# e4s2022/e4s

Measured on AMD Instinct MI355X. Metric: 1024^2 face-swap images/sec, higher is better.
Workload: dtype f32 operands as hi+lo bf16, 3 bf16 MFMAs per product, f32 accumulate (bf16x3) on the 3x3 convs whose launch fills the chip; exact f32 elsewhere; 1 GPU; E4S-core face swap at 1024^2 (2x Net3 encoder @256^2, style swap, 12 LocalMLPs, mask-guided StyleGAN2 generator K=13), BASELINE.json configs[3] shard: 8 swaps per GPU per step; per_gpu_batch=8, global_batch=8, out_size=1024, hip_graph=True, precision=as bf16x3 where the launch fills the chip (this batch), else exact fp32, parallelism=image-parallel x1

## Files before the change

e4s_amd/build.py:

```python
import hashlib
import os
import subprocess
import sys

HERE = os.path.dirname(os.path.abspath(__file__))
ROOT = os.path.dirname(HERE)
CSRC = os.path.join(HERE, "csrc")
LIB = os.path.join(HERE, "libe4s_hip.so")
STAMP = os.path.join(HERE, ".libe4s_hip.stamp")
ARCH = "gfx950"


def sources():
    return sorted(os.path.join(CSRC, f) for f in os.listdir(CSRC) if f.endswith(".hip"))


PER_FILE_FLAGS = {"conv_region1w.hip": ["-fno-slp-vectorize"], "conv_wino1w.hip": ["-fno-slp-vectorize"],
                  "conv_gather1w.hip": ["-fno-slp-vectorize"]}


def _extra_flags():
    flags = ["-DE4S_ABLATIONS"] if os.environ.get("E4S_BUILD_ABLATIONS") == "1" else []
    return flags + os.environ.get("E4S_EXTRA_CFLAGS", "").split()


def _digest():
    h = hashlib.sha256()
    h.update(" ".join(_extra_flags()).encode())
    h.update(repr(sorted(PER_FILE_FLAGS.items())).encode())
    headers = sorted(os.path.join(CSRC, f) for f in os.listdir(CSRC) if f.endswith(".h"))
    files = sources() + headers + [os.path.join(ROOT, "include", "e4s_hip.h")]
    for f in files:
        h.update(f.encode())
        with open(f, "rb") as fh:
            h.update(fh.read())
    return h.hexdigest()


def _compile_and_link(lib, objdir, verbose):
    hipcc = os.environ.get("HIPCC", "/opt/rocm/bin/hipcc")
    if not os.path.isfile(hipcc):
        hipcc = "hipcc"
    os.makedirs(objdir, exist_ok=True)
    procs, objs = [], []
    for src in sources():
        obj = os.path.join(objdir, os.path.basename(src) + ".o")
        cmd = [hipcc, f"--offload-arch={ARCH}", "-O3", "-std=c++17", "-fPIC", "-I" + os.path.join(ROOT, "include"),
               "-I" + CSRC] + _extra_flags() + PER_FILE_FLAGS.get(os.path.basename(src), []) + ["-c", src, "-o", obj]
        if verbose:
            print(" ".join(cmd), flush=True)
        procs.append((src, subprocess.Popen(cmd, stdout=subprocess.PIPE, stderr=subprocess.STDOUT)))
        objs.append(obj)
    for src, pr in procs:
        out, _ = pr.communicate()
        if pr.returncode != 0:
            sys.stderr.write(out.decode(errors="replace"))
            raise RuntimeError(f"hipcc failed on {src}")
    res = subprocess.run([hipcc, f"--offload-arch={ARCH}", "-shared", "-fPIC", "-o", lib] + objs, stdout=subprocess.PIPE, stderr=subprocess.STDOUT)
    if res.returncode != 0:
        sys.stderr.write(res.stdout.decode(errors="replace"))
        raise RuntimeError(f"link of {os.path.basename(lib)} failed")
    return lib


def build(force=False, verbose=False):
    alt = os.environ.get("E4S_BUILD_OUT")
    if alt:
        return _build_to(os.path.abspath(alt), os.path.join(os.path.dirname(os.path.abspath(alt)), "obj_" + os.path.basename(alt)), verbose)
    dig = _digest()
    if not force and os.path.isfile(LIB) and os.path.isfile(STAMP) and open(STAMP).read().strip() == dig:
        return LIB
    _compile_and_link(LIB, os.path.join(HERE, "build"), verbose)
    with open(STAMP, "w") as fh:
        fh.write(dig)
    return LIB


def _build_to(lib, objdir, verbose=False):
    return _compile_and_link(lib, objdir, verbose)


if __name__ == "__main__":
    print(build(force="--force" in sys.argv, verbose=True))
```

e4s_amd/csrc/upconv_bf16x3.hip:

```cpp
#include "conv_launch.h"
#include <stdlib.h>

namespace {


constexpr int PKC = 32;
constexpr int KC = 16, ROWB = 80, LO = 32;
constexpr int TAH = 8, TAW = 16;
constexpr int HH = TAH + 1, HW = TAW + 1, HALO = HH * HW;
constexpr int OH = 2 * TAH - 4, OW = 2 * TAW - 4;
constexpr int IQH = 2 * TAH, IQW = 2 * TAW;
constexpr int BNC = 32;
constexpr int NTHR = 256, NBLK = 9;
constexpr int ITEMS = HALO * 2;
constexpr int AJ = (ITEMS + NTHR - 1) / NTHR;
constexpr int BPIECES = NBLK * BNC * 4;
constexpr int BJ = (BPIECES + NTHR - 1) / NTHR;
constexpr int A_BYTES = HALO * ROWB;
constexpr int B_BYTES = NBLK * BNC * ROWB;
constexpr int STAGE_BYTES = 2 * A_BYTES + 2 * B_BYTES;
constexpr int I_BYTES = IQH * IQW * BNC * 4;
constexpr int NZ = OH * OW;
constexpr int MAXC = 512;
constexpr int SMEM = STAGE_BYTES + NZ * 4 + 2 * MAXC * 4;
static_assert(I_BYTES <= STAGE_BYTES, "the I tile aliases the stage buffers");
static_assert(2 * SMEM <= 160 * 1024, "two blocks per CU");
static_assert(8 * OW <= NTHR && NZ <= 2 * NTHR, "epilogue thread layout");

__device__ __forceinline__ void split_store(unsigned char* dst, const f32x8 v) {
    const bf16x8 h = __builtin_convertvector(v, bf16x8);
    const f32x8 r = v - __builtin_convertvector(h, f32x8);
    const bf16x8 l = __builtin_convertvector(r, bf16x8);
    *reinterpret_cast<bf16x8*>(dst) = h;
    *reinterpret_cast<bf16x8*>(dst + LO) = l;
}

struct TileId { int tb, ty, tx, nt; };

template <int XF, int PC = 0>
__global__ __launch_bounds__(NTHR, 2) void upconv_fused_kernel(const e4s_conv_params p, const float* __restrict__ k4, const int ntn,
                                                           const int tx_n, const int per_img, const int ntiles, const int abl_arg) {
#ifdef E4S_ABLATIONS
    const int abl = abl_arg;
#else
    constexpr int abl = 0;
#endif
    extern __shared__ __attribute__((aligned(16))) unsigned char smem[];
    unsigned char* sA = smem;
    unsigned char* sB = smem + 2 * A_BYTES;
    float* sI = reinterpret_cast<float*>(smem);
    float* s_nz = reinterpret_cast<float*>(smem + STAGE_BYTES);
    float* s_sty = s_nz + NZ;

    const int tid = threadIdx.x;
    const int lane = tid & 63, wm = __builtin_amdgcn_readfirstlane(tid >> 6);
    const int li = lane & 31, kh = lane >> 5;
    const int G = gridDim.x;
    const int first = xcd_remap(blockIdx.x, G);
    const int nchunk = p.Cin / KC;
    const unsigned char* wbytes = reinterpret_cast<const unsigned char*>(p.w);
    const size_t img_stride = (size_t)p.Hi * p.Wi * p.Cin;

    auto decode = [&](int t) -> TileId {
        TileId id;
        const int mt = t / ntn;
        id.nt = t - mt * ntn;
        id.tb = mt / per_img;
        const int rem = mt - id.tb * per_img;
        id.ty = rem / tx_n;
        id.tx = rem - id.ty * tx_n;
        return id;
    };
    auto item_src = [&](const TileId& id, int item, bool& ok) -> size_t {
        const int h = item >> 1, q = item & 1;
        const int hy = h / HW, hx = h - hy * HW;
        const int iy = id.ty * (OH / 2) - 2 + hy, ix = id.tx * (OW / 2) - 2 + hx;
        ok = item < ITEMS && (unsigned)iy < (unsigned)p.Hi && (unsigned)ix < (unsigned)p.Wi;
        return ok ? ((size_t)iy * p.Wi + ix) * p.Cin + q * 8 : (size_t)(q * 8);
    };
    auto item_dst = [&](int item) -> int { return (item >> 1) * ROWB + (item & 1) * 16; };
    const f32x8 zero8 = {0.f, 0.f, 0.f, 0.f, 0.f, 0.f, 0.f, 0.f};
    auto b_src = [&](int i, int c, int nt) -> size_t {
        return ((size_t)(c >> 1) * ntn + nt) * (NBLK * BNC * 128) + (size_t)(i >> 2) * 128 + ((i >> 1) & 1) * 64 + (c & 1) * 32 + (i & 1) * 16;
    };
    auto b_dst = [&](int i) -> int { return (i >> 2) * ROWB + (i & 3) * 16; };

    struct AReg {
        f32x8 a[AJ];
        bool ok[AJ];
    };
    typedef f32x4 BReg[BJ];
    auto fetch_a = [&](AReg& R, const TileId& id, int chunk, bool real) {
        const float* xb = p.x + (real ? (size_t)id.tb * img_stride + chunk * KC : 0);
#pragma unroll
        for (int j = 0; j < AJ; ++j) {
            const int item = tid + NTHR * j;
            const size_t off = item_src(id, item, R.ok[j]);
            if (abl != 4) R.a[j] = load8(xb + off);
        }
    };
    auto load_style = [&](const TileId& id, int par) {
        if (XF)
            for (int i = tid * 4; i < p.Cin; i += NTHR * 4)
                *reinterpret_cast<f32x4*>(s_sty + par * MAXC + i) = *reinterpret_cast<const f32x4*>(p.in_scale + (size_t)id.tb * p.Cin + i);
    };
    auto fetch_b = [&](BReg& R, const TileId& id, int chunk, bool real) {
#pragma unroll
        for (int j = 0; j < BJ; ++j) {
            const int i = tid + NTHR * j;
            if (abl != 4) R[j] = *reinterpret_cast<const f32x4*>(wbytes + b_src(i < BPIECES ? i : 0, real ? chunk : 0, real ? id.nt : 0));
        }
    };
    auto store_a = [&](const AReg& R, int buf, int chunk, int par) {
#pragma unroll
        for (int j = 0; j < AJ; ++j) {
            const int item = tid + NTHR * j;
            if (item < ITEMS) {
                f32x8 v = R.a[j];
                if (XF) v = v * load8(s_sty + par * MAXC + chunk * KC + (item & 1) * 8);
                if (!R.ok[j]) v = zero8;
                split_store(sA + buf * A_BYTES + item_dst(item), v);
            }
        }
    };
    auto store_b = [&](const BReg& R, int buf) {
#pragma unroll
        for (int j = 0; j < BJ; ++j) {
            const int i = tid + NTHR * j;
            if (i < BPIECES) *reinterpret_cast<f32x4*>(sB + buf * B_BYTES + b_dst(i)) = R[j];
        }
    };

    if (first >= ntiles) return;
    TileId cur = decode(first);
    int t_next = first + G;
    bool has_next = t_next < ntiles;
    TileId nxt = decode(has_next ? t_next : first);

    AReg RE, RO;
    BReg RB;
    int par = 0;
    fetch_a(RE, cur, 0, true);
    fetch_b(RB, cur, 0, true);
    load_style(cur, 0);
    if (XF) __syncthreads();
    store_a(RE, 0, 0, 0);
    store_b(RB, 0);
    fetch_a(RO, cur, 1, true);
    __syncthreads();

    const int m_row = wm * 32 + li;
    const int arow = ((m_row / TAW) * HW + (m_row % TAW)) * ROWB + kh * 16;
    const int brow = li * ROWB + kh * 16;
    const int e_c4 = tid & 7, e_ox = tid >> 3;
    const bool e_act = e_ox < OW;

    float fu[4], fv[4];
    bool sep;
    {
        float kk[16], vmax = 0.f;
#pragma unroll
        for (int a = 0; a < 16; ++a) {
            kk[a] = k4[a];
            vmax = fmaxf(vmax, fabsf(kk[a]));
        }
        sep = kk[0] != 0.f;
        const float inv = sep ? 1.f / kk[0] : 0.f;
#pragma unroll
        for (int i = 0; i < 4; ++i) {
            fu[3 - i] = kk[4 * i];
            fv[3 - i] = kk[i] * inv;
        }
#pragma unroll
        for (int i = 0; i < 4; ++i)
#pragma unroll
            for (int j = 0; j < 4; ++j) sep = sep && fabsf(kk[4 * i + j] - fu[3 - i] * fv[3 - j]) <= 1e-6f * vmax;
    }

    f32x16 acc[4];
    auto contract = [&](int buf) {
        const unsigned char* Ab = sA + buf * A_BYTES + arow;
        const unsigned char* Bb = sB + buf * B_BYTES + brow;
        struct Frag { bf16x8 h, l; };
        auto ldA = [&](int shift) -> Frag {
            const unsigned char* a = Ab + ((1 - (shift >> 1)) * HW + (1 - (shift & 1))) * ROWB;
            return Frag{*reinterpret_cast<const bf16x8*>(a), *reinterpret_cast<const bf16x8*>(a + LO)};
        };
        auto ldB = [&](int blk) -> Frag {
            const unsigned char* b = Bb + blk * (BNC * ROWB);
            return Frag{*reinterpret_cast<const bf16x8*>(b), *reinterpret_cast<const bf16x8*>(b + LO)};
        };
        {
            const Frag a0 = ldA(0), b0 = ldB(0), b4 = ldB(4), b6 = ldB(6), b8 = ldB(8);
            const Frag a1 = ldA(1), b1 = ldB(1), b7 = ldB(7);
            acc[0] = __builtin_amdgcn_mfma_f32_32x32x16_bf16(a0.l, b0.h, acc[0], 0, 0, 0);
            acc[1] = __builtin_amdgcn_mfma_f32_32x32x16_bf16(a0.l, b4.h, acc[1], 0, 0, 0);
            acc[2] = __builtin_amdgcn_mfma_f32_32x32x16_bf16(a0.l, b6.h, acc[2], 0, 0, 0);
            acc[3] = __builtin_amdgcn_mfma_f32_32x32x16_bf16(a0.l, b8.h, acc[3], 0, 0, 0);
            acc[0] = __builtin_amdgcn_mfma_f32_32x32x16_bf16(a0.h, b0.l, acc[0], 0, 0, 0);
            acc[1] = __builtin_amdgcn_mfma_f32_32x32x16_bf16(a0.h, b4.l, acc[1], 0, 0, 0);
            acc[2] = __builtin_amdgcn_mfma_f32_32x32x16_bf16(a0.h, b6.l, acc[2], 0, 0, 0);
            acc[3] = __builtin_amdgcn_mfma_f32_32x32x16_bf16(a0.h, b8.l, acc[3], 0, 0, 0);
            acc[0] = __builtin_amdgcn_mfma_f32_32x32x16_bf16(a0.h, b0.h, acc[0], 0, 0, 0);
            acc[1] = __builtin_amdgcn_mfma_f32_32x32x16_bf16(a0.h, b4.h, acc[1], 0, 0, 0);
            acc[2] = __builtin_amdgcn_mfma_f32_32x32x16_bf16(a0.h, b6.h, acc[2], 0, 0, 0);
            acc[3] = __builtin_amdgcn_mfma_f32_32x32x16_bf16(a0.h, b8.h, acc[3], 0, 0, 0);
            acc[0] = __builtin_amdgcn_mfma_f32_32x32x16_bf16(a1.l, b1.h, acc[0], 0, 0, 0);
            acc[2] = __builtin_amdgcn_mfma_f32_32x32x16_bf16(a1.l, b7.h, acc[2], 0, 0, 0);
            acc[0] = __builtin_amdgcn_mfma_f32_32x32x16_bf16(a1.h, b1.l, acc[0], 0, 0, 0);
            acc[2] = __builtin_amdgcn_mfma_f32_32x32x16_bf16(a1.h, b7.l, acc[2], 0, 0, 0);
            acc[0] = __builtin_amdgcn_mfma_f32_32x32x16_bf16(a1.h, b1.h, acc[0], 0, 0, 0);
            acc[2] = __builtin_amdgcn_mfma_f32_32x32x16_bf16(a1.h, b7.h, acc[2], 0, 0, 0);
        }
        {
            const Frag a2 = ldA(2), b2 = ldB(2), b5 = ldB(5);
            const Frag a3 = ldA(3), b3 = ldB(3);
            acc[0] = __builtin_amdgcn_mfma_f32_32x32x16_bf16(a2.l, b2.h, acc[0], 0, 0, 0);
            acc[1] = __builtin_amdgcn_mfma_f32_32x32x16_bf16(a2.l, b5.h, acc[1], 0, 0, 0);
            acc[0] = __builtin_amdgcn_mfma_f32_32x32x16_bf16(a2.h, b2.l, acc[0], 0, 0, 0);
            acc[1] = __builtin_amdgcn_mfma_f32_32x32x16_bf16(a2.h, b5.l, acc[1], 0, 0, 0);
            acc[0] = __builtin_amdgcn_mfma_f32_32x32x16_bf16(a2.h, b2.h, acc[0], 0, 0, 0);
            acc[1] = __builtin_amdgcn_mfma_f32_32x32x16_bf16(a2.h, b5.h, acc[1], 0, 0, 0);
            acc[0] = __builtin_amdgcn_mfma_f32_32x32x16_bf16(a3.l, b3.h, acc[0], 0, 0, 0);
            acc[0] = __builtin_amdgcn_mfma_f32_32x32x16_bf16(a3.h, b3.l, acc[0], 0, 0, 0);
            acc[0] = __builtin_amdgcn_mfma_f32_32x32x16_bf16(a3.h, b3.h, acc[0], 0, 0, 0);
        }
    };

    for (;;) {
        if (has_next) load_style(nxt, par ^ 1);
#pragma unroll
        for (int c = 0; c < 4; ++c)
#pragma unroll
            for (int r = 0; r < 16; ++r) acc[c][r] = 0.f;
        float nz_reg[2] = {0.f, 0.f};
        if (!PC && p.noise) {
#pragma unroll
            for (int j = 0; j < 2; ++j) {
                const int e = tid + NTHR * j;
                const int oy = cur.ty * OH + e / OW, ox = cur.tx * OW + e % OW;
                if (e < NZ && oy < p.Ho && ox < p.Wo) nz_reg[j] = p.noise[(int64_t)cur.tb * p.noise_bstride + (int64_t)oy * p.Wo + ox];
            }
        }
        f32x4 d_reg = {1.f, 1.f, 1.f, 1.f}, b_reg = {0.f, 0.f, 0.f, 0.f};
        if (e_act) {
            const int co0 = cur.nt * BNC + e_c4 * 4;
            if (p.out_scale) d_reg = *reinterpret_cast<const f32x4*>(p.out_scale + (size_t)cur.tb * p.Cout + co0);
            if (p.bias) b_reg = *reinterpret_cast<const f32x4*>(p.bias + co0);
        }
        const float nw_reg = p.noise ? p.noise_w[0] : 0.f;

        for (int c0 = 0; c0 < nchunk; c0 += 2) {
            const bool last_pair = (c0 + 2 == nchunk);
            const TileId& nid = last_pair ? nxt : cur;
            const bool nreal = !last_pair || has_next;
            const int ce = last_pair ? 0 : c0 + 2, co = last_pair ? 1 : c0 + 3;
            fetch_a(RE, nid, ce, nreal);
            fetch_b(RB, cur, c0 + 1, true);
            if (abl != 1) contract(0);
            if (abl != 5) {
                store_a(RO, 1, c0 + 1, par);
                store_b(RB, 1);
            }
            __syncthreads();
            fetch_a(RO, nid, co, nreal);
            fetch_b(RB, nid, ce, nreal);
            if (abl != 1) contract(1);
            if (!last_pair && abl != 5) {
                store_a(RE, 0, ce, par);
                store_b(RB, 0);
            }
            __syncthreads();
        }

#pragma unroll
        for (int j = 0; j < 2; ++j)
            if (!PC && tid + NTHR * j < NZ) s_nz[tid + NTHR * j] = nw_reg * nz_reg[j];
        if (abl == 3 || abl == 7) asm volatile("" :: "v"(acc[0][0]), "v"(acc[1][7]), "v"(acc[2][3]), "v"(acc[3][9]));
        if (abl != 3 && abl != 7)
#pragma unroll
        for (int cls = 0; cls < 4; ++cls) {
            const int dy = cls >> 1, dx = cls & 1;
#pragma unroll
            for (int r = 0; r < 16; ++r) {
                const int m = wm * 32 + (r & 3) + 8 * (r >> 2) + 4 * kh;
                const int qy = 2 * (m / TAW) + dy, qx = 2 * (m % TAW) + dx;
                sI[(qy * IQW + qx) * BNC + li] = acc[cls][r];
            }
        }
        __syncthreads();
        if (e_act && abl != 2 && abl != 3) {
            const int co0 = cur.nt * BNC + e_c4 * 4;
            const int ox = cur.tx * OW + e_ox;
            const f32x4 d = d_reg, bs = b_reg;
            const float gain = (p.act == 1) ? p.gain : 1.f;
            const int ycs = p.y_cstride ? p.y_cstride : p.Cout;
            const float* ip = sI + (IQW + e_ox + 1) * BNC + e_c4 * 4;
            auto finish = [&](f32x4 v, int r) {
                const int oy = cur.ty * OH + r;
                if (oy < p.Ho && ox < p.Wo) {
                    if (PC) {
                        const f32x4 nz = *reinterpret_cast<const f32x4*>(
                            p.noise + ((int64_t)cur.tb * p.noise_bstride + (int64_t)oy * p.Wo + ox) * p.Cout + co0);
                        f32x4 nzw;
#pragma unroll
                        for (int e = 0; e < 4; ++e) nzw[e] = e4s_mul_rn(nw_reg, nz[e]);
                        v = v * d + bs + nzw;
                    } else
                    v = v * d + bs + s_nz[r * OW + e_ox];
                    if (p.act) {
#pragma unroll
                        for (int e = 0; e < 4; ++e) v[e] = (v[e] > 0.f ? v[e] : v[e] * p.alpha) * gain;
                    }
                    f32x4* dst = reinterpret_cast<f32x4*>(p.y + (((size_t)cur.tb * p.Ho + oy) * p.Wo + ox) * ycs + co0);
                    if (abl == 6) asm volatile("" :: "v"(v));
                    else *dst = v;
                }
            };
            if (sep) {
                auto hrow = [&](int ry) -> f32x4 {
                    const float* q = ip + ry * IQW * BNC;
                    return *reinterpret_cast<const f32x4*>(q) * fv[0] + *reinterpret_cast<const f32x4*>(q + BNC) * fv[1] +
                           *reinterpret_cast<const f32x4*>(q + 2 * BNC) * fv[2] + *reinterpret_cast<const f32x4*>(q + 3 * BNC) * fv[3];
                };
                f32x4 h0 = hrow(0), h1 = hrow(1), h2 = hrow(2);
#pragma unroll
                for (int r = 0; r < OH; ++r) {
                    const f32x4 h3 = hrow(r + 3);
                    finish(h0 * fu[0] + h1 * fu[1] + h2 * fu[2] + h3 * fu[3], r);
                    h0 = h1;
                    h1 = h2;
                    h2 = h3;
                }
            } else {
                float kf[16];
#pragma unroll
                for (int a = 0; a < 16; ++a) kf[a] = k4[15 - a];
                f32x4 win[3][4];
#pragma unroll
                for (int ry = 0; ry < 3; ++ry)
#pragma unroll
                    for (int ax = 0; ax < 4; ++ax) win[ry][ax] = *reinterpret_cast<const f32x4*>(ip + (ry * IQW + ax) * BNC);
#pragma unroll
                for (int r = 0; r < OH; ++r) {
                    f32x4 nw[4];
#pragma unroll
                    for (int ax = 0; ax < 4; ++ax) nw[ax] = *reinterpret_cast<const f32x4*>(ip + ((r + 3) * IQW + ax) * BNC);
                    f32x4 v = {0.f, 0.f, 0.f, 0.f};
#pragma unroll
                    for (int ax = 0; ax < 4; ++ax)
                        v += win[0][ax] * kf[ax] + win[1][ax] * kf[4 + ax] + win[2][ax] * kf[8 + ax] + nw[ax] * kf[12 + ax];
#pragma unroll
                    for (int ax = 0; ax < 4; ++ax) { win[0][ax] = win[1][ax]; win[1][ax] = win[2][ax]; win[2][ax] = nw[ax]; }
                    finish(v, r);
                }
            }
        }
        if (!has_next) break;
        __syncthreads();
        if (abl != 5) {
            store_a(RE, 0, 0, par ^ 1);
            store_b(RB, 0);
        }
        __syncthreads();
        cur = nxt;
        par ^= 1;
        t_next += G;
        has_next = t_next < ntiles;
        if (has_next) nxt = decode(t_next);
    }
}

__global__ void subpixel_weights_kernel(const float* __restrict__ w, unsigned short* __restrict__ out, int Cout, int Cin,
                                        int64_t n8) {
    const int64_t i = (int64_t)blockIdx.x * blockDim.x + threadIdx.x;
    if (i >= n8) return;
    const int q = (int)(i & 3);
    int64_t r = i >> 2;
    const int col = (int)(r % BNC); r /= BNC;
    const int blk = (int)(r % NBLK); r /= NBLK;
    const int ntn = Cout / BNC;
    const int nt = (int)(r % ntn), chunk = (int)(r / ntn);
    const int cls_of[9] = {0, 0, 0, 0, 1, 1, 2, 2, 3}, sh_of[9] = {0, 1, 2, 3, 0, 2, 0, 1, 0};
    const int cls = cls_of[blk], s = sh_of[blk];
    const int ky = (cls >> 1) + 2 * (s >> 1), kx = (cls & 1) + 2 * (s & 1);
    const int co = nt * BNC + col, ci0 = chunk * PKC + q * 8;
    f32x8 v;
#pragma unroll
    for (int e = 0; e < 8; ++e) v[e] = w[(((size_t)co * Cin + ci0 + e) * 3 + ky) * 3 + kx];
    const bf16x8 h = __builtin_convertvector(v, bf16x8);
    const f32x8 res = v - __builtin_convertvector(h, f32x8);
    const bf16x8 l = __builtin_convertvector(res, bf16x8);
    unsigned short* d = out + (i >> 2) * 64 + q * 8;
    *reinterpret_cast<bf16x8*>(d) = h;
    *reinterpret_cast<bf16x8*>(d + 32) = l;
}

}

extern "C" int e4s_subpixel_weights_f32(const float* w, void* out, int Cout, int Cin, void* stream) {
    if (Cout % BNC || Cin % PKC || Cout <= 0 || Cin <= 0) return (int)hipErrorInvalidValue;
    const int64_t n8 = (int64_t)(Cin / PKC) * (Cout / BNC) * NBLK * BNC * 4;
    hipLaunchKernelGGL(subpixel_weights_kernel, dim3(cdiv(n8, 256)), dim3(256), 0, as_stream(stream), w,
                       reinterpret_cast<unsigned short*>(out), Cout, Cin, n8);
    E4S_CHECK_LAUNCH();
    return 0;
}

extern "C" int e4s_upconv_bf16x3_f32(const e4s_conv_params* pp, const float* k4, void* stream) {
    const e4s_conv_params& p = *pp;
    if (p.Cin % (2 * KC) || p.Cin > MAXC || p.Cout % BNC || !k4 || p.labels || p.tiles || p.in_stats || p.act == 2 ||
        p.Ho != 2 * p.Hi || p.Wo != 2 * p.Wi || p.B <= 0 || (p.y_cstride && p.y_cstride % 4))
        return (int)hipErrorInvalidValue;
    hipStream_t st = as_stream(stream);
    const bool pc = p.noise && p.noise_per_channel;
    if (pc && (!p.in_scale || !p.noise_w || !aligned16(p.noise) || (p.noise_bstride != 0 && p.noise_bstride != (int64_t)p.Ho * p.Wo)))
        return (int)hipErrorInvalidValue;
    auto kern = pc ? upconv_fused_kernel<1, 1> : p.in_scale ? upconv_fused_kernel<1, 0> : upconv_fused_kernel<0, 0>;
    static std::atomic<uint64_t> smem_set0{0}, smem_set1{0}, smem_set2{0};
    if (int e = e4s_ensure_dyn_smem(reinterpret_cast<const void*>(kern), SMEM, pc ? smem_set2 : p.in_scale ? smem_set1 : smem_set0)) return e;
    const int ntn = p.Cout / BNC;
    const int tx_n = (p.Wo + OW - 1) / OW, per_img = ((p.Ho + OH - 1) / OH) * tx_n;
    const int64_t ntiles = (int64_t)p.B * per_img * ntn;
    if (ntiles >= (1ll << 31)) return (int)hipErrorInvalidValue;
    const int slots = 2 * e4s_num_cus();
    const int grid = (int)(ntiles < slots ? ntiles : slots);
    int abl = 0;
#ifdef E4S_ABLATIONS
    if (const char* e = getenv("E4S_UPCONV3_ABL")) abl = atoi(e);
#endif
    hipLaunchKernelGGL(kern, dim3((unsigned)grid), dim3(NTHR), SMEM, st, p, k4, ntn, tx_n, per_img, (int)ntiles, abl);
    E4S_CHECK_LAUNCH();
    return 0;
}
```

Before: 517.7 images/s.

## Add one-wave-per-tile upsample conv kernel with register-resident weight fragments

Adds a new bf16x3 fused upsample-conv kernel for large launches. Each wave independently owns an output tile, holds all nine weight blocks in registers as MFMA fragments, and uses wave-private LDS with wave-level fences instead of block barriers. It also interleaves A stores and B loads with the MFMAs through sched_group_barrier. The subpixel weight packing is rewritten into a lane-major 64-lane fragment layout so B loads are direct 16-byte per-lane reads, and the old kernel's b_src indexing is updated to match. The dispatcher picks the new path when there are at least three tiles per CU, and it runs at one wave per EU, trading occupancy for register reuse.

```diff
diff --git a/e4s_amd/build.py b/e4s_amd/build.py
--- a/e4s_amd/build.py
+++ b/e4s_amd/build.py
@@ -16,7 +16,7 @@
 
 
 PER_FILE_FLAGS = {"conv_region1w.hip": ["-fno-slp-vectorize"], "conv_wino1w.hip": ["-fno-slp-vectorize"],
-                  "conv_gather1w.hip": ["-fno-slp-vectorize"]}
+                  "conv_gather1w.hip": ["-fno-slp-vectorize"], "upconv_bf16x3_1w.hip": ["-fno-slp-vectorize"]}
 
 
 def _extra_flags():
diff --git a/e4s_amd/csrc/upconv_bf16x3.hip b/e4s_amd/csrc/upconv_bf16x3.hip
--- a/e4s_amd/csrc/upconv_bf16x3.hip
+++ b/e4s_amd/csrc/upconv_bf16x3.hip
@@ -1,4 +1,5 @@
 #include "conv_launch.h"
+#include "upconv_bf16x3_1w.h"
 #include <stdlib.h>
 
 namespace {
@@ -23,6 +24,7 @@
 constexpr int NZ = OH * OW;
 constexpr int MAXC = 512;
 constexpr int SMEM = STAGE_BYTES + NZ * 4 + 2 * MAXC * 4;
+constexpr int ONE_WAVE_MIN_TILES_PER_CU = 3;
 static_assert(I_BYTES <= STAGE_BYTES, "the I tile aliases the stage buffers");
 static_assert(2 * SMEM <= 160 * 1024, "two blocks per CU");
 static_assert(8 * OW <= NTHR && NZ <= 2 * NTHR, "epilogue thread layout");
@@ -81,7 +83,7 @@
     auto item_dst = [&](int item) -> int { return (item >> 1) * ROWB + (item & 1) * 16; };
     const f32x8 zero8 = {0.f, 0.f, 0.f, 0.f, 0.f, 0.f, 0.f, 0.f};
     auto b_src = [&](int i, int c, int nt) -> size_t {
-        return ((size_t)(c >> 1) * ntn + nt) * (NBLK * BNC * 128) + (size_t)(i >> 2) * 128 + ((i >> 1) & 1) * 64 + (c & 1) * 32 + (i & 1) * 16;
+        return ((((size_t)c * ntn + nt) * NBLK + (i >> 7)) * 2 + ((i >> 1) & 1)) * 1024 + ((i & 1) * 32 + ((i >> 2) & 31)) * 16;
     };
     auto b_dst = [&](int i) -> int { return (i >> 2) * ROWB + (i & 3) * 16; };
 
@@ -375,32 +377,31 @@
                                         int64_t n8) {
     const int64_t i = (int64_t)blockIdx.x * blockDim.x + threadIdx.x;
     if (i >= n8) return;
-    const int q = (int)(i & 3);
-    int64_t r = i >> 2;
-    const int col = (int)(r % BNC); r /= BNC;
+    const int lane = (int)(i & 63);
+    int64_t r = i >> 6;
     const int blk = (int)(r % NBLK); r /= NBLK;
     const int ntn = Cout / BNC;
     const int nt = (int)(r % ntn), chunk = (int)(r / ntn);
     const int cls_of[9] = {0, 0, 0, 0, 1, 1, 2, 2, 3}, sh_of[9] = {0, 1, 2, 3, 0, 2, 0, 1, 0};
     const int cls = cls_of[blk], s = sh_of[blk];
     const int ky = (cls >> 1) + 2 * (s >> 1), kx = (cls & 1) + 2 * (s & 1);
-    const int co = nt * BNC + col, ci0 = chunk * PKC + q * 8;
+    const int co = nt * BNC + (lane & 31), ci0 = chunk * KC + (lane >> 5) * 8;
     f32x8 v;
 #pragma unroll
     for (int e = 0; e < 8; ++e) v[e] = w[(((size_t)co * Cin + ci0 + e) * 3 + ky) * 3 + kx];
     const bf16x8 h = __builtin_convertvector(v, bf16x8);
     const f32x8 res = v - __builtin_convertvector(h, f32x8);
     const bf16x8 l = __builtin_convertvector(res, bf16x8);
-    unsigned short* d = out + (i >> 2) * 64 + q * 8;
+    unsigned short* d = out + (i >> 6) * 1024 + lane * 8;
     *reinterpret_cast<bf16x8*>(d) = h;
-    *reinterpret_cast<bf16x8*>(d + 32) = l;
+    *reinterpret_cast<bf16x8*>(d + 512) = l;
 }
 
 }
 
 extern "C" int e4s_subpixel_weights_f32(const float* w, void* out, int Cout, int Cin, void* stream) {
     if (Cout % BNC || Cin % PKC || Cout <= 0 || Cin <= 0) return (int)hipErrorInvalidValue;
-    const int64_t n8 = (int64_t)(Cin / PKC) * (Cout / BNC) * NBLK * BNC * 4;
+    const int64_t n8 = (int64_t)(Cin / KC) * (Cout / BNC) * NBLK * 64;
     hipLaunchKernelGGL(subpixel_weights_kernel, dim3(cdiv(n8, 256)), dim3(256), 0, as_stream(stream), w,
                        reinterpret_cast<unsigned short*>(out), Cout, Cin, n8);
     E4S_CHECK_LAUNCH();
@@ -416,6 +417,14 @@
     const bool pc = p.noise && p.noise_per_channel;
     if (pc && (!p.in_scale || !p.noise_w || !aligned16(p.noise) || (p.noise_bstride != 0 && p.noise_bstride != (int64_t)p.Ho * p.Wo)))
         return (int)hipErrorInvalidValue;
+    {
+        int tx1, per1;
+        const int n1 = e4s_upconv1w_tiles(p, &tx1, &per1);
+        bool one_wave = n1 >= ONE_WAVE_MIN_TILES_PER_CU * e4s_num_cus();
+        if (const char* e = getenv("E4S_UPCONV_1W")) one_wave = atoi(e) != 0;
+        one_wave = one_wave && n1 >= 0 && e4s_upconv1w_ok(p);
+        if (one_wave) return e4s_launch_upconv1w(p, k4, st);
+    }
     auto kern = pc ? upconv_fused_kernel<1, 1> : p.in_scale ? upconv_fused_kernel<1, 0> : upconv_fused_kernel<0, 0>;
     static std::atomic<uint64_t> smem_set0{0}, smem_set1{0}, smem_set2{0};
     if (int e = e4s_ensure_dyn_smem(reinterpret_cast<const void*>(kern), SMEM, pc ? smem_set2 : p.in_scale ? smem_set1 : smem_set0)) return e;
diff --git a/e4s_amd/csrc/upconv_bf16x3_1w.h b/e4s_amd/csrc/upconv_bf16x3_1w.h
--- /dev/null
+++ b/e4s_amd/csrc/upconv_bf16x3_1w.h
@@ -0,0 +1,15 @@
+#pragma once
+#include "common.h"
+
+namespace upconv1w {
+constexpr int KC = 16;
+constexpr int TAH = 16, TAW = 8;
+constexpr int HH = TAH + 1, HW = TAW + 1;
+constexpr int OH = 2 * TAH - 4, OW = 2 * TAW - 4;
+constexpr int BNC = 32;
+constexpr int NBLK = 9;
+}
+
+int e4s_upconv1w_tiles(const e4s_conv_params& p, int* tx_n, int* per_img);
+bool e4s_upconv1w_ok(const e4s_conv_params& p);
+int e4s_launch_upconv1w(const e4s_conv_params& p, const float* k4, hipStream_t st);
diff --git a/e4s_amd/csrc/upconv_bf16x3_1w.hip b/e4s_amd/csrc/upconv_bf16x3_1w.hip
--- /dev/null
+++ b/e4s_amd/csrc/upconv_bf16x3_1w.hip
@@ -0,0 +1,491 @@
+#include "conv_launch.h"
+#include "upconv_bf16x3_1w.h"
+#include <stdlib.h>
+#include <type_traits>
+
+namespace {
+
+using namespace upconv1w;
+
+constexpr int ROWB = 80, LO = 32;
+constexpr int HALO = HH * HW;
+constexpr int NTHR = 256, WAVES = 4;
+constexpr int ITEMS = HALO * 2;
+constexpr int AJ = (ITEMS + 63) / 64;
+constexpr int A_BYTES = AJ * 32 * ROWB;
+constexpr int NZ = OH * OW;
+constexpr int NZJ = (NZ + 63) / 64;
+constexpr int WAVE_BYTES = 2 * A_BYTES + NZ * 4;
+constexpr int SMEM = WAVES * WAVE_BYTES;
+constexpr int FRAG = 64 * 16;
+static_assert(WAVE_BYTES % 16 == 0, "wave-private LDS slices stay 16-byte aligned");
+
+typedef unsigned u32x2 __attribute__((ext_vector_type(2)));
+
+struct Frag { bf16x8 h, l; };
+struct TileId { int tb, ty, tx, nt; };
+
+__device__ __forceinline__ void wave_lds_fence() {
+    __builtin_amdgcn_fence(__ATOMIC_RELEASE, "wavefront", "local");
+    __builtin_amdgcn_wave_barrier();
+    __builtin_amdgcn_fence(__ATOMIC_ACQUIRE, "wavefront", "local");
+}
+
+__device__ __forceinline__ void split_store(unsigned char* dst, const f32x8 v) {
+    const bf16x8 h = __builtin_convertvector(v, bf16x8);
+    const f32x8 r = v - __builtin_convertvector(h, f32x8);
+    const bf16x8 l = __builtin_convertvector(r, bf16x8);
+    *reinterpret_cast<bf16x8*>(dst) = h;
+    *reinterpret_cast<bf16x8*>(dst + LO) = l;
+}
+
+template <int XF, int PC, int ABL = 0>
+__global__ __launch_bounds__(NTHR) __attribute__((amdgpu_waves_per_eu(1, 1)))
+void upconv1w_kernel(const e4s_conv_params p, const float* __restrict__ k4, const int ntn, const int tx_n, const int per_img,
+                     const int ntiles) {
+    constexpr int abl = ABL;
+    extern __shared__ __attribute__((aligned(16))) unsigned char smem[];
+    const int tid = threadIdx.x;
+    const int lane = tid & 63, wv = __builtin_amdgcn_readfirstlane(tid >> 6);
+    const int li = lane & 31, kh = lane >> 5;
+    unsigned char* sA = smem + wv * WAVE_BYTES;
+    float* s_nz = reinterpret_cast<float*>(sA + 2 * A_BYTES);
+    const int G = gridDim.x;
+    const int nchunk = p.Cin / KC;
+    const unsigned char* wbytes = reinterpret_cast<const unsigned char*>(p.w);
+    const unsigned lane16 = lane * 16;
+    const int64_t img_stride = (int64_t)p.Hi * p.Wi * p.Cin;
+
+    auto decode = [&](int t) -> TileId {
+        TileId id;
+        const int mt = t / ntn;
+        id.nt = t - mt * ntn;
+        id.tb = mt / per_img;
+        const int rem = mt - id.tb * per_img;
+        id.ty = rem / tx_n;
+        id.tx = rem - id.ty * tx_n;
+        return id;
+    };
+
+    const int q8 = (lane & 1) * 8;
+    unsigned rel[AJ];
+    int hyx[AJ];
+#pragma unroll
+    for (int j = 0; j < AJ; ++j) {
+        const int item = lane + 64 * j, h = item >> 1;
+        hyx[j] = (item < ITEMS ? h / HW : (1 << 15)) << 8 | (h % HW);
+        rel[j] = item < ITEMS ? (unsigned)(((h / HW) * p.Wi + h % HW) * p.Cin + q8) * 4u : 0u;
+    }
+    const int a_dst = (lane >> 1) * ROWB + (lane & 1) * 16;
+    const f32x8 zero8 = {0.f, 0.f, 0.f, 0.f, 0.f, 0.f, 0.f, 0.f};
+
+    struct AReg {
+        f32x8 a[AJ], sty;
+        bool ok[AJ];
+    };
+    auto fetch_a = [&](AReg& R, const TileId& id, int chunk, bool real) {
+        if (abl == 1 || abl == 2) return;
+        const int y0 = id.ty * (OH / 2) - 2, x0 = id.tx * (OW / 2) - 2;
+        const unsigned char* xs = reinterpret_cast<const unsigned char*>(p.x + (real ? (int64_t)id.tb * img_stride : 0));
+        const unsigned org = (unsigned)((y0 * p.Wi + x0) * p.Cin + chunk * KC) * 4u;
+#pragma unroll
+        for (int j = 0; j < AJ; ++j) {
+            R.ok[j] = real & ((unsigned)(y0 + (hyx[j] >> 8)) < (unsigned)p.Hi) & ((unsigned)(x0 + (hyx[j] & 255)) < (unsigned)p.Wi);
+            R.a[j] = load8(reinterpret_cast<const float*>(xs + (R.ok[j] ? org + rel[j] : (unsigned)q8 * 4u)));
+        }
+    };
+    auto fetch_sty = [&](AReg& R, const TileId& id, int chunk, bool real) {
+        if (abl == 1 || abl == 2) return;
+        if (XF) R.sty = load8(reinterpret_cast<const float*>(
+                    reinterpret_cast<const unsigned char*>(p.in_scale + (real ? (int64_t)id.tb * p.Cin + chunk * KC : 0)) + (unsigned)q8 * 4u));
+    };
+    auto store_item = [&](const AReg& R, int buf, int j) {
+        if (abl == 1 || abl == 2) return;
+        f32x8 v = R.a[j];
+        if (XF) {
+#pragma unroll
+            for (int e = 0; e < 8; ++e) v[e] *= R.sty[e];
+        }
+        if (!R.ok[j]) v = zero8;
+        split_store(sA + buf * A_BYTES + a_dst + j * 32 * ROWB, v);
+    };
+    auto interleave = [&](auto n, auto nv) {
+#pragma unroll
+        for (int i = 0; i < decltype(n)::value; ++i) {
+            __builtin_amdgcn_sched_group_barrier(0x008, 1, 0);
+            __builtin_amdgcn_sched_group_barrier(0x002, decltype(nv)::value, 0);
+        }
+    };
+
+    const int a_row = ((li >> 3) * HW + (li & 7)) * ROWB + kh * 16;
+    auto ldA = [&](Frag (&a)[4], int buf, int t) {
+        if (abl == 1) return;
+        const unsigned char* Ab = sA + buf * A_BYTES + a_row;
+#pragma unroll
+        for (int s = 0; s < 4; ++s) {
+            const unsigned char* q = Ab + ((4 * t + 1 - (s >> 1)) * HW + 1 - (s & 1)) * ROWB;
+            a[s].h = *reinterpret_cast<const bf16x8*>(q);
+            a[s].l = *reinterpret_cast<const bf16x8*>(q + LO);
+        }
+    };
+    Frag B[NBLK];
+    const unsigned char* wnext = wbytes;
+    auto ldB = [&](int blk) {
+        if (abl == 1 || abl == 3) return;
+        B[blk].h = *reinterpret_cast<const bf16x8*>(wnext + blk * 2 * FRAG + lane16);
+        B[blk].l = *reinterpret_cast<const bf16x8*>(wnext + blk * 2 * FRAG + FRAG + lane16);
+    };
+    auto stage_image = [&](const TileId& id, int chunk, bool real) -> const unsigned char* {
+        return wbytes + (real ? ((size_t)chunk * ntn + id.nt) * (NBLK * 2 * FRAG) : 0);
+    };
+
+    const int first = xcd_remap(blockIdx.x, G) * WAVES + wv;
+    if (first >= ntiles) return;
+    TileId cur = decode(first);
+    int64_t t_next = (int64_t)first + (int64_t)G * WAVES;
+    bool has_next = t_next < ntiles;
+    TileId nxt = decode(has_next ? (int)t_next : first);
+
+    float fu[4], fv[4];
+    bool sep;
+    {
+        float kk[16], vmax = 0.f;
+#pragma unroll
+        for (int a = 0; a < 16; ++a) {
+            kk[a] = k4[a];
+            vmax = fmaxf(vmax, fabsf(kk[a]));
+        }
+        sep = kk[0] != 0.f;
+        const float inv = sep ? 1.f / kk[0] : 0.f;
+#pragma unroll
+        for (int i = 0; i < 4; ++i) {
+            fu[3 - i] = kk[4 * i];
+            fv[3 - i] = kk[i] * inv;
+        }
+#pragma unroll
+        for (int i = 0; i < 4; ++i)
+#pragma unroll
+            for (int j = 0; j < 4; ++j) sep = sep && fabsf(kk[4 * i + j] - fu[3 - i] * fv[3 - j]) <= 1e-6f * vmax;
+    }
+
+    f32x16 acc[4][4];
+#define E4S_MM(A_, B_, C_) C_ = __builtin_amdgcn_mfma_f32_32x32x16_bf16(A_, B_, C_, 0, 0, 0)
+    auto grp0 = [&](const Frag (&a)[4], int t) {
+        E4S_MM(a[0].l, B[0].h, acc[t][0]); E4S_MM(a[0].l, B[4].h, acc[t][1]); E4S_MM(a[0].l, B[6].h, acc[t][2]); E4S_MM(a[0].l, B[8].h, acc[t][3]);
+        E4S_MM(a[0].h, B[0].l, acc[t][0]); E4S_MM(a[0].h, B[4].l, acc[t][1]); E4S_MM(a[0].h, B[6].l, acc[t][2]); E4S_MM(a[0].h, B[8].l, acc[t][3]);
+        E4S_MM(a[0].h, B[0].h, acc[t][0]); E4S_MM(a[0].h, B[4].h, acc[t][1]); E4S_MM(a[0].h, B[6].h, acc[t][2]); E4S_MM(a[0].h, B[8].h, acc[t][3]);
+    };
+    auto grp1 = [&](const Frag (&a)[4], int t) {
+        E4S_MM(a[1].l, B[1].h, acc[t][0]); E4S_MM(a[1].l, B[7].h, acc[t][2]);
+        E4S_MM(a[1].h, B[1].l, acc[t][0]); E4S_MM(a[1].h, B[7].l, acc[t][2]);
+        E4S_MM(a[1].h, B[1].h, acc[t][0]); E4S_MM(a[1].h, B[7].h, acc[t][2]);
+    };
+    auto grp2 = [&](const Frag (&a)[4], int t) {
+        E4S_MM(a[2].l, B[2].h, acc[t][0]); E4S_MM(a[2].l, B[5].h, acc[t][1]);
+        E4S_MM(a[2].h, B[2].l, acc[t][0]); E4S_MM(a[2].h, B[5].l, acc[t][1]);
+        E4S_MM(a[2].h, B[2].h, acc[t][0]); E4S_MM(a[2].h, B[5].h, acc[t][1]);
+    };
+    auto grp3 = [&](const Frag (&a)[4], int t) {
+        E4S_MM(a[3].l, B[3].h, acc[t][0]);
+        E4S_MM(a[3].h, B[3].l, acc[t][0]);
+        E4S_MM(a[3].h, B[3].h, acc[t][0]);
+    };
+#undef E4S_MM
+    auto mtile = [&](const Frag (&a)[4], int t) {
+        grp0(a, t);
+        grp1(a, t);
+        grp2(a, t);
+        grp3(a, t);
+    };
+
+    AReg RA;
+    Frag A0[4], A1[4];
+    if (abl == 1 || abl == 3) {
+#pragma unroll
+        for (int b = 0; b < NBLK; ++b) B[b].h = B[b].l = *reinterpret_cast<const bf16x8*>(wbytes + lane16);
+    }
+    if (abl == 1) {
+#pragma unroll
+        for (int s = 0; s < 4; ++s) A0[s].h = A0[s].l = A1[s].h = A1[s].l = *reinterpret_cast<const bf16x8*>(wbytes + FRAG + lane16);
+    }
+    fetch_a(RA, cur, 0, true);
+    fetch_sty(RA, cur, 0, true);
+    wnext = stage_image(cur, 0, true);
+#pragma unroll
+    for (int b = 0; b < NBLK; ++b) ldB(b);
+#pragma unroll
+    for (int j = 0; j < AJ; ++j) store_item(RA, 0, j);
+    wave_lds_fence();
+    ldA(A0, 0, 0);
+    int buf = 0;
+
+    const int c4 = li & ~3;
+    for (;;) {
+#pragma unroll
+        for (int t = 0; t < 4; ++t)
+#pragma unroll
+            for (int c = 0; c < 4; ++c)
+#pragma unroll
+                for (int r = 0; r < 16; ++r) acc[t][c][r] = 0.f;
+        int lane_t = lane;
+        asm volatile("" : "+v"(lane_t));
+        float nz_reg[NZJ];
+#pragma unroll
+        for (int j = 0; j < NZJ; ++j) {
+            nz_reg[j] = 0.f;
+            if (!PC && p.noise) {
+                const int e = lane_t + 64 * j;
+                const int oy = cur.ty * OH + e / OW, ox = cur.tx * OW + e % OW;
+                if (e < NZ && oy < p.Ho && ox < p.Wo) nz_reg[j] = p.noise[(int64_t)cur.tb * p.noise_bstride + (int64_t)oy * p.Wo + ox];
+            }
+        }
+        const float nw_reg = p.noise ? p.noise_w[0] : 0.f;
+
+        for (int c = 0; c < nchunk; ++c) {
+            const bool last = (c + 1 == nchunk);
+            const TileId& nid = last ? nxt : cur;
+            const bool nreal = !last || has_next;
+            const int cn = last ? 0 : c + 1;
+            fetch_a(RA, nid, cn, nreal);
+            wnext = stage_image(nid, cn, nreal);
+            __builtin_amdgcn_sched_barrier(0);
+            ldA(A1, buf, 1);
+            __builtin_amdgcn_sched_barrier(0);
+            mtile(A0, 0);
+            __builtin_amdgcn_sched_barrier(0);
+            if (!PC && c == 0) {
+#pragma unroll
+                for (int j = 0; j < NZJ; ++j)
+                    if (lane_t + 64 * j < NZ) s_nz[lane_t + 64 * j] = nw_reg * nz_reg[j];
+            }
+            ldA(A0, buf, 2);
+            __builtin_amdgcn_sched_barrier(0);
+            mtile(A1, 1);
+            __builtin_amdgcn_sched_barrier(0);
+            ldA(A1, buf, 3);
+            fetch_sty(RA, nid, cn, nreal);
+            __builtin_amdgcn_sched_barrier(0);
+            mtile(A0, 2);
+            __builtin_amdgcn_sched_barrier(0);
+            store_item(RA, buf ^ 1, 0);
+            store_item(RA, buf ^ 1, 1);
+            grp0(A1, 3);
+            interleave(std::integral_constant<int, 12>{}, std::integral_constant<int, 8>{});
+            __builtin_amdgcn_sched_barrier(0);
+            if (!last) { ldB(0); ldB(4); ldB(6); ldB(8); }
+            store_item(RA, buf ^ 1, 2);
+            grp1(A1, 3);
+            interleave(std::integral_constant<int, 6>{}, std::integral_constant<int, 8>{});
+            __builtin_amdgcn_sched_barrier(0);
+            if (!last) { ldB(1); ldB(7); }
+            store_item(RA, buf ^ 1, 3);
+            grp2(A1, 3);
+            interleave(std::integral_constant<int, 6>{}, std::integral_constant<int, 8>{});
+            __builtin_amdgcn_sched_barrier(0);
+            if (!last) { ldB(2); ldB(5); }
+            store_item(RA, buf ^ 1, 4);
+            grp3(A1, 3);
+            __builtin_amdgcn_sched_barrier(0);
+            if (!last) ldB(3);
+            wave_lds_fence();
+            if (!last) ldA(A0, buf ^ 1, 0);
+            __builtin_amdgcn_sched_barrier(0);
+            buf ^= 1;
+        }
+
+        const int co0 = cur.nt * BNC + c4;
+        f32x4 d_reg = {1.f, 1.f, 1.f, 1.f}, b_reg = {0.f, 0.f, 0.f, 0.f};
+        if (p.out_scale) d_reg = *reinterpret_cast<const f32x4*>(p.out_scale + (size_t)cur.tb * p.Cout + co0);
+        if (p.bias) b_reg = *reinterpret_cast<const f32x4*>(p.bias + co0);
+        auto next_tile_b = [&]() {
+#pragma unroll
+            for (int b = 0; b < NBLK; ++b) ldB(b);
+        };
+        constexpr int QY_NEXT_B = 20;
+        if (abl == 1 || abl == 4) {
+#pragma unroll
+            for (int t = 0; t < 4; ++t) asm volatile("" :: "v"(acc[t][0][0]), "v"(acc[t][1][7]), "v"(acc[t][2][3]), "v"(acc[t][3][9]));
+            next_tile_b();
+        } else {
+            const float gain = (p.act == 1) ? p.gain : 1.f;
+            const int ycs = p.y_cstride ? p.y_cstride : p.Cout;
+            const int rows_left = p.Ho - cur.ty * OH, cols_left = p.Wo - cur.tx * OW;
+            int lane_e = lane;
+            asm volatile("" : "+v"(lane_e));
+            const int i4 = lane_e & 3, c4 = lane_e & 28;
+            const int oxh = (OW / 2) * (lane_e >> 5);
+            const int oxA = oxh + i4, oxB = oxh + (i4 < 2 ? 4 + i4 : i4 - 2), oxC = oxh + 2 + i4, rowB = i4 >> 1;
+            const bool okA = oxA < cols_left, okB = oxB < cols_left, okC = oxC < cols_left;
+            const int64_t pix0 = ((int64_t)cur.tb * p.Ho + cur.ty * OH) * p.Wo + cur.tx * OW;
+            unsigned char* ytile = reinterpret_cast<unsigned char*>(p.y + pix0 * ycs + cur.nt * BNC);
+            const unsigned yrow = (unsigned)p.Wo * ycs * 4u;
+            const unsigned yA = (unsigned)(oxA * ycs + c4) * 4u, yB = (unsigned)((rowB * p.Wo + oxB) * ycs + c4) * 4u,
+                           yC = (unsigned)((p.Wo + oxC) * ycs + c4) * 4u;
+            const unsigned char* ntile = nullptr;
+            unsigned nrow = 0, nA = 0, nB = 0, nC = 0;
+            if (PC) {
+                ntile = reinterpret_cast<const unsigned char*>(
+                    p.noise + ((int64_t)cur.tb * p.noise_bstride + ((int64_t)cur.ty * OH * p.Wo + cur.tx * OW)) * p.Cout + cur.nt * BNC);
+                nrow = (unsigned)p.Wo * p.Cout * 4u;
+                nA = (unsigned)(oxA * p.Cout + c4) * 4u;
+                nB = (unsigned)((rowB * p.Wo + oxB) * p.Cout + c4) * 4u;
+                nC = (unsigned)((p.Wo + oxC) * p.Cout + c4) * 4u;
+            }
+            const int zA = oxA, zB = rowB * OW + oxB, zC = OW + oxC;
+            auto finish = [&](const float a0, const float a1, const float a2, const float a3, const int r0, const bool ok,
+                              const unsigned yoff, const unsigned noff, const int zoff) {
+                if (ok) {
+                    float v[4] = {a0, a1, a2, a3};
+                    if (PC) {
+                        const f32x4 nz = *reinterpret_cast<const f32x4*>((ntile + (size_t)r0 * nrow) + noff);
+#pragma unroll
+                        for (int e = 0; e < 4; ++e) v[e] = v[e] * d_reg[e] + b_reg[e] + e4s_mul_rn(nw_reg, nz[e]);
+                    } else {
+                        const float nz = s_nz[r0 * OW + zoff];
+#pragma unroll
+                        for (int e = 0; e < 4; ++e) v[e] = v[e] * d_reg[e] + b_reg[e] + nz;
+                    }
+                    if (p.act) {
+#pragma unroll
+                        for (int e = 0; e < 4; ++e) v[e] = (v[e] > 0.f ? v[e] : v[e] * p.alpha) * gain;
+                    }
+                    const f32x4 o = {v[0], v[1], v[2], v[3]};
+                    if (abl == 5) asm volatile("" :: "v"(o));
+                    else *reinterpret_cast<f32x4*>((ytile + (size_t)r0 * yrow) + yoff) = o;
+                }
+            };
+            auto emit = [&](const int r0, const float (&e)[6], const float (&o)[6]) {
+                if (r0 >= rows_left) return;
+                float a0 = e[0], a1 = e[1], a2 = e[2], a3 = e[3];
+                quad_transpose4(a0, a1, a2, a3, lane);
+                finish(a0, a1, a2, a3, r0, okA, yA, nA, zA);
+                a0 = e[4]; a1 = e[5]; a2 = o[0]; a3 = o[1];
+                quad_transpose4(a0, a1, a2, a3, lane);
+                finish(a0, a1, a2, a3, r0, okB, yB, nB, zB);
+                a0 = o[2]; a1 = o[3]; a2 = o[4]; a3 = o[5];
+                quad_transpose4(a0, a1, a2, a3, lane);
+                finish(a0, a1, a2, a3, r0, okC, yC, nC, zC);
+            };
+            auto window = [&](float (&w)[9], const int qy) {
+                float c[8];
+#pragma unroll
+                for (int k = 0; k < 8; ++k) c[k] = acc[qy >> 3][2 * (qy & 1) + (k & 1)][4 * ((qy >> 1) & 3) + (k >> 1)];
+                const u32x2 s1 = __builtin_amdgcn_permlane32_swap(__float_as_uint(c[0]), __float_as_uint(c[7]), false, false);
+                const u32x2 s2 = __builtin_amdgcn_permlane32_swap(__float_as_uint(c[1]), __float_as_uint(c[1]), false, false);
+                const float x7 = __uint_as_float(s1[0]), x8 = __uint_as_float(s1[1]), x9 = __uint_as_float(s2[1]);
+                w[0] = kh ? x7 : c[1];
+#pragma unroll
+                for (int j = 1; j < 7; ++j) w[j] = kh ? c[j - 1] : c[j + 1];
+                w[7] = kh ? c[6] : x8;
+                w[8] = kh ? c[7] : x9;
+            };
+            float ev[6];
+            if (sep) {
+                float H[4][6];
+#pragma unroll
+                for (int qy = 1; qy < 2 * TAH; ++qy) {
+                    float w[9];
+                    window(w, qy);
+#pragma unroll
+                    for (int j = 0; j < 6; ++j) H[(qy - 1) & 3][j] = w[j] * fv[0] + w[j + 1] * fv[1] + w[j + 2] * fv[2] + w[j + 3] * fv[3];
+                    if (qy >= 4) {
+                        const int r = qy - 4;
+                        float o[6];
+#pragma unroll
+                        for (int j = 0; j < 6; ++j)
+                            o[j] = H[r & 3][j] * fu[0] + H[(r + 1) & 3][j] * fu[1] + H[(r + 2) & 3][j] * fu[2] + H[(r + 3) & 3][j] * fu[3];
+                        if (r & 1) emit(r - 1, ev, o);
+                        else {
+#pragma unroll
+                            for (int j = 0; j < 6; ++j) ev[j] = o[j];
+                        }
+                    }
+                    __builtin_amdgcn_sched_barrier(0);
+                    if (qy == QY_NEXT_B) {
+                        next_tile_b();
+                        __builtin_amdgcn_sched_barrier(0);
+                    }
+                }
+            } else {
+                float kf[16];
+#pragma unroll
+                for (int a = 0; a < 16; ++a) kf[a] = k4[15 - a];
+                float W[4][9];
+#pragma unroll
+                for (int qy = 1; qy < 2 * TAH; ++qy) {
+                    window(W[(qy - 1) & 3], qy);
+                    if (qy >= 4) {
+                        const int r = qy - 4;
+                        float o[6];
+#pragma unroll
+                        for (int j = 0; j < 6; ++j) {
+                            float v = 0.f;
+#pragma unroll
+                            for (int ax = 0; ax < 4; ++ax)
+                                v += W[r & 3][j + ax] * kf[ax] + W[(r + 1) & 3][j + ax] * kf[4 + ax] + W[(r + 2) & 3][j + ax] * kf[8 + ax] +
+                                     W[(r + 3) & 3][j + ax] * kf[12 + ax];
+                            o[j] = v;
+                        }
+                        if (r & 1) emit(r - 1, ev, o);
+                        else {
+#pragma unroll
+                            for (int j = 0; j < 6; ++j) ev[j] = o[j];
+                        }
+                    }
+                    __builtin_amdgcn_sched_barrier(0);
+                    if (qy == QY_NEXT_B) {
+                        next_tile_b();
+                        __builtin_amdgcn_sched_barrier(0);
+                    }
+                }
+            }
+        }
+        if (!has_next) break;
+        ldA(A0, buf, 0);
+        cur = nxt;
+        t_next += (int64_t)G * WAVES;
+        has_next = t_next < ntiles;
+        if (has_next) nxt = decode((int)t_next);
+    }
+}
+
+}
+
+bool e4s_upconv1w_ok(const e4s_conv_params& p) {
+    const int64_t cs = p.y_cstride > p.Cout ? p.y_cstride : p.Cout;
+    return (int64_t)(OH + 1) * p.Wo * cs * 4 < (1ll << 31) && (int64_t)p.Hi * p.Wi * p.Cin * 4 < (1ll << 31);
+}
+
+int e4s_upconv1w_tiles(const e4s_conv_params& p, int* tx_n, int* per_img) {
+    *tx_n = (p.Wo + OW - 1) / OW;
+    *per_img = ((p.Ho + OH - 1) / OH) * *tx_n;
+    const int64_t n = (int64_t)p.B * *per_img * (p.Cout / BNC);
+    return n >= (1ll << 31) ? -1 : (int)n;
+}
+
+int e4s_launch_upconv1w(const e4s_conv_params& p, const float* k4, hipStream_t st) {
+    const bool pc = p.noise && p.noise_per_channel;
+    auto kern = pc ? upconv1w_kernel<1, 1> : p.in_scale ? upconv1w_kernel<1, 0> : upconv1w_kernel<0, 0>;
+    int slot = pc ? 2 : p.in_scale ? 1 : 0;
+#ifdef E4S_ABLATIONS
+    if (const char* e = getenv("E4S_UPCONV3_ABL")) {
+        const int a = atoi(e);
+        if (a >= 1 && a <= 5 && !pc && p.in_scale) {
+            decltype(kern) tab[5] = {upconv1w_kernel<1, 0, 1>, upconv1w_kernel<1, 0, 2>, upconv1w_kernel<1, 0, 3>, upconv1w_kernel<1, 0, 4>,
+                                     upconv1w_kernel<1, 0, 5>};
+            kern = tab[a - 1];
+            slot = 2 + a;
+        }
+    }
+#endif
+    static std::atomic<uint64_t> smem_set[8];
+    if (int e = e4s_ensure_dyn_smem(reinterpret_cast<const void*>(kern), SMEM, smem_set[slot])) return e;
+    int tx_n, per_img;
+    const int ntiles = e4s_upconv1w_tiles(p, &tx_n, &per_img);
+    if (ntiles < 0) return (int)hipErrorInvalidValue;
+    const int blocks = (ntiles + WAVES - 1) / WAVES, cus = e4s_num_cus();
+    const int grid = blocks < cus ? blocks : cus;
+    hipLaunchKernelGGL(kern, dim3((unsigned)grid), dim3(NTHR), SMEM, st, p, k4, p.Cout / BNC, tx_n, per_img, ntiles);
+    E4S_CHECK_LAUNCH();
+    return 0;
+}
```

After: 522.0 images/s, median of 6. No clear change (+0.8%).
